# Rengar-Yang/humanoid-gym-with-comments

Measured on AMD Instinct MI355X. Metric: env-steps/sec (whole node) at 4096 envs + PPO iters/sec, 1/2/4/8 MI355X, higher is better.
Workload: dtype f32; 1 GPU; XBot-L flat terrain, 4096 envs/GPU, PPO 24-step rollout (BASELINE configs[1]); envs_per_gpu=4096, num_steps_per_env=24, parallelism=dp1, ppo=2 epochs x 4 minibatches, actor 705-512-256-128-12, critic 219-768-256-128-1, update_graph=one, gemm_table=tuning/tunableop_mi355x_f32.csv

## Files before the change

humanoid-gym-with-comments_amd/csrc/hg_gemm.hip:

```cpp
#include <hip/hip_runtime.h>
#include <stdint.h>

#include <type_traits>

#include "hg_common.h"

namespace {

typedef float f32x16 __attribute__((ext_vector_type(16)));
typedef float f32x4u __attribute__((ext_vector_type(4), aligned(4)));

struct GemmArgs {
  const float* A;
  int64_t lda;
  const float* B;
  int64_t ldb;
  const float* bias;
  const float* Y;
  int64_t ldY;
  float* C;
  int64_t ldc;
  float* colpart;
  int64_t M;
  int N, K;
// ... 676 lines not shown
    epi_input_grad<TM, TN, ELU>(acc, g, m0 + wm0, n0 + wn0, i, h, cs);
#pragma unroll
    for (int n = 0; n < TN; n++) {
      const int cl = wn0 + 32 * n + i;
      cs[n] += __shfl_xor(cs[n], 32);
      if (h == 0) red[(wave % WGM) * BN + cl] = cs[n];
    }
    if (g.colpart) {
      __syncthreads();
      for (int c = tid; c < BN; c += NT) {
        if (n0 + c <= nmax) {
          float sum = 0.f;
#pragma unroll
          for (int w = 0; w < WGM; w++) sum += red[w * BN + c];
          g.colpart[tm_idx * g.N + n0 + c] = sum;
        }
      }
    }
  }
}

template <int BM, int BN, int WGM, int WGN, int KG, bool VEC, int MODE, bool ELU, int IMG = 0, bool APF = false>
__global__ void __launch_bounds__(64 * WGM * WGN) k_gemm_x6(GemmX6Args xa) {
  gemm_x6_body<BM, BN, WGM, WGN, KG, VEC, MODE, ELU, IMG, APF>(xa);
}

template <int BM, int BN, int WGM, int WGN, int KG, bool VEC, int MODE, bool ELU, int IMG = 0, bool APF = false,
          int OCC = 4>
__global__ void __launch_bounds__(64 * WGM * WGN) __attribute__((amdgpu_waves_per_eu(OCC)))
k_gemm_x6_occ(GemmX6Args xa) {
  gemm_x6_body<BM, BN, WGM, WGN, KG, VEC, MODE, ELU, IMG, APF>(xa);
}

constexpr int IMG_MAX = 16;
struct ImageJobs {
  const float* P[IMG_MAX];
  bf16x8* img[IMG_MAX];
  int64_t ld[IMG_MAX], pitch[IMG_MAX];
  int trans[IMG_MAX], R[IMG_MAX], K[IMG_MAX], groups[IMG_MAX];
  int block0[IMG_MAX + 1];
  int njobs;
};

__host__ __device__ inline int64_t img_rows(int64_t R) { return (R + 255) / 256 * 256; }
__host__ __device__ inline int64_t img_chunks(int64_t K) { return (K + 31) / 32 * 2; }

__global__ void __launch_bounds__(256) k_x6_image_jobs(ImageJobs J) {
  const int bid = blockIdx.x;
  int j = 0;
  while (j + 1 < J.njobs && bid >= J.block0[j + 1]) j++;
  const int lb = bid - J.block0[j];
  const int grp = lb % J.groups[j], c = lb / J.groups[j];
  const int r = grp * 128 + (threadIdx.x & 127), h = threadIdx.x >> 7;
  const float* __restrict__ P = J.P[j];
  const int64_t ld = J.ld[j];
  const int R = J.R[j], K = J.K[j];
  const int k0 = c * 16 + 8 * h;
  float v[8];
  if (J.trans[j]) {
#pragma unroll
    for (int q = 0; q < 8; q++) v[q] = (r < R && k0 + q < K) ? P[(int64_t)(k0 + q) * ld + r] : 0.f;
  } else if (r < R && k0 + 8 <= K && ld % 4 == 0 && ((uintptr_t)P & 15) == 0) {
    const float4 a = *reinterpret_cast<const float4*>(P + (int64_t)r * ld + k0);
    const float4 b = *reinterpret_cast<const float4*>(P + (int64_t)r * ld + k0 + 4);
    v[0] = a.x; v[1] = a.y; v[2] = a.z; v[3] = a.w; v[4] = b.x; v[5] = b.y; v[6] = b.z; v[7] = b.w;
  } else {
// ... 21 lines not shown
#define HG_X6I(V, MD, E, I)                                                                                      \
  do {                                                                                                             \
    if constexpr (OCC > 0) hipLaunchKernelGGL((k_gemm_x6_occ<BM, BN, WGM, WGN, KG, V, MD, E, I, APF, OCC>), grid, block, 0, s, xa); \
    else hipLaunchKernelGGL((k_gemm_x6<BM, BN, WGM, WGN, KG, V, MD, E, I, APF>), grid, block, 0, s, xa);             \
  } while (0)
  if (mode == 2) {
    HG_X6I(false, 2, false, 3);
  } else if (mode == 4) {
    if (vec) HG_X6I(true, 4, false, 1);
    else HG_X6I(false, 4, false, 1);
  } else if (img == 3) {
    if (mode == 0) {
      if (elu) HG_X6I(false, 0, true, 3);
      else HG_X6I(false, 0, false, 3);
    } else {
      if (elu) HG_X6I(false, 1, true, 3);
      else HG_X6I(false, 1, false, 3);
    }
  } else if (mode == 0) {
    if (vec && elu) HG_X6I(true, 0, true, 1);
    else if (vec) HG_X6I(true, 0, false, 1);
    else if (elu) HG_X6I(false, 0, true, 1);
    else HG_X6I(false, 0, false, 1);
  } else {
    if (vec && elu) HG_X6I(true, 1, true, 1);
    else if (vec) HG_X6I(true, 1, false, 1);
    else if (elu) HG_X6I(false, 1, true, 1);
    else HG_X6I(false, 1, false, 1);
  }
#undef HG_X6I
  return hipGetLastError() == hipSuccess ? HG_OK : HG_ERR_HIP;
}

int x6_img_dispatch(int tile, int mode, int img, GemmX6Args xa, bool vec, bool elu, hipStream_t s) {
  switch (tile) {
    case 20: return launch_x6_img<128, 128, 2, 2, 1>(mode, img, xa, vec, elu, s);
    case 21: return launch_x6_img<128, 128, 2, 4, 1>(mode, img, xa, vec, elu, s);
    case 22: return launch_x6_img<128, 64, 2, 2, 1>(mode, img, xa, vec, elu, s);
    case 23: return launch_x6_img<64, 64, 2, 2, 1>(mode, img, xa, vec, elu, s);
    case 24: return launch_x6_img<128, 128, 2, 2, 2>(mode, img, xa, vec, elu, s);
    case 25: return launch_x6_img<256, 128, 4, 2, 1>(mode, img, xa, vec, elu, s);
    case 26: return launch_x6_img<128, 128, 2, 4, 2>(mode, img, xa, vec, elu, s);
    case 27: return launch_x6_img<128, 256, 2, 4, 1>(mode, img, xa, vec, elu, s);
    case 28: return launch_x6_img<64, 256, 2, 4, 1>(mode, img, xa, vec, elu, s);
    case 29: return launch_x6_img<64, 64, 2, 2, 1, true>(mode, img, xa, vec, elu, s);
    case 30: return launch_x6_img<256, 128, 4, 2, 1, false, 4>(mode, img, xa, vec, elu, s);
    case 31: return launch_x6_img<128, 64, 2, 2, 1, false, 4>(mode, img, xa, vec, elu, s);
    case 32: return launch_x6_img<128, 128, 2, 4, 1, false, 6>(mode, img, xa, vec, elu, s);
    default: return launch_x6_img<64, 128, 2, 2, 1>(mode, img, xa, vec, elu, s);
  }
}

template <int BM, int BN, int WGM, int WGN, int KG>
int launch_x6(int mode, GemmX6Args xa, bool vec, bool elu, hipStream_t s) {
  GemmArgs& g = xa.g;
  g.tiles_n = (g.N + BN - 1) / BN;
  const int64_t tiles_m = (g.M + BM - 1) / BM;
  g.tiles = tiles_m * g.tiles_n;
  if (mode != 2 && mode != 4) xa.slices = 1;
  if (g.tiles * xa.slices > 0x7fffffff) return HG_ERR_ARG;
  const dim3 grid((unsigned)(g.tiles * xa.slices)), block(64 * WGM * WGN);
#define HG_X6(V, MD, E) hipLaunchKernelGGL((k_gemm_x6<BM, BN, WGM, WGN, KG, V, MD, E>), grid, block, 0, s, xa)
  if (mode == 0) {
    if (vec && elu) HG_X6(true, 0, true);
    else if (vec) HG_X6(true, 0, false);
    else if (elu) HG_X6(false, 0, true);
    else HG_X6(false, 0, false);
  } else if (mode == 1) {
    if (vec && elu) HG_X6(true, 1, true);
    else if (vec) HG_X6(true, 1, false);
    else if (elu) HG_X6(false, 1, true);
    else HG_X6(false, 1, false);
  } else if (mode == 3) {
    if (vec && elu) HG_X6(true, 3, true);
    else if (vec) HG_X6(true, 3, false);
    else if (elu) HG_X6(false, 3, true);
    else HG_X6(false, 3, false);
  } else if (mode == 4) {
    if (vec) HG_X6(true, 4, false);
    else HG_X6(false, 4, false);
  } else {
    HG_X6(false, 2, false);
  }
#undef HG_X6
  return hipGetLastError() == hipSuccess ? HG_OK : HG_ERR_HIP;
}

constexpr int NTILES = 29;
constexpr int NTILES_IMG = 32;
int tile_bm(int tile) {
  if (tile == 25 || tile == 30) return 256;
  return (tile <= 2 || (tile >= 8 && tile <= 10) || tile == 12 || tile == 13 || tile == 16 || tile == 17 ||
          (tile >= 20 && tile <= 22) || tile == 24 || tile == 26 || tile == 27 || tile == 31 || tile == 32)
             ? 128
             : 64;
}

struct WgradArgs {
  const float* A;
  int64_t lda;
  const float* B;
  int64_t ldb;
  float* C;
  int64_t ldc, cstride;
  int M, N;
  int64_t R, kslice;
  int slices, tiles_n;
  int64_t tiles;
};

typedef short s16x4 __attribute__((ext_vector_type(4)));
typedef float f32x2 __attribute__((ext_vector_type(2)));
typedef __bf16 bf16x2 __attribute__((ext_vector_type(2)));

__device__ __forceinline__ uint32_t bf16_pair(f32x2 v) {
  return __builtin_bit_cast(uint32_t, __builtin_convertvector(v, bf16x2));
}
__device__ __forceinline__ f32x2 bf16_pair_f32(uint32_t u) {
  f32x2 r;
  r[0] = __uint_as_float(u << 16);
  r[1] = __uint_as_float(u & 0xffff0000u);
  return r;
}
__device__ __forceinline__ void split3x4(const float v[4], uint2& p0, uint2& p1, uint2& p2) {
// ... 209 lines not shown
    J.pitch[j] = img_rows(prow) * 2;
    J.trans[j] = trans[j];
    J.R[j] = (int)rows[j];
    J.K[j] = (int)K[j];
    J.groups[j] = (int)(img_rows(rows[j]) / 128);
    J.block0[j] = (int)blocks;
    blocks += img_chunks(K[j]) * J.groups[j];
    if (blocks > (int64_t)1 << 30) return HG_ERR_ARG;
  }
  J.block0[njobs] = (int)blocks;
  for (int j = 0; j < njobs;) {
    const int64_t prow = pitch_rows && pitch_rows[j] > 0 ? pitch_rows[j] : rows[j];
    int64_t sum = rows[j];
    int e = j + 1;
    while (e < njobs && pitch_rows && pitch_rows[e] == prow && K[e] == K[j] && sum < prow &&
           (uintptr_t)img[e] == (uintptr_t)img[e - 1] + (uintptr_t)(32 * rows[e - 1])) {
      sum += rows[e];
      e++;
    }
    if (sum != prow) return HG_ERR_ARG;
    for (int b = j; b + 1 < e; b++)
      if (rows[b] % 256) return HG_ERR_ARG;
    j = e;
  }
  hipLaunchKernelGGL(k_x6_image_jobs, dim3((unsigned)blocks), dim3(256), 0, (hipStream_t)stream, J);
  return hipGetLastError() == hipSuccess ? HG_OK : HG_ERR_HIP;
}

extern "C" int hg_gemm_f32_img(int mode, const float* A, int64_t lda, const void* Aimg, const void* Bimg,
                               const float* bias, const float* Y, int64_t ldY, float* C, int64_t ldc, float* colpart,
                               int64_t M, int N, int K, int act, int tile, int64_t aimg_bytes, int64_t bimg_bytes,
                               void* stream) {
  if ((!A && !Aimg) || !Bimg || !C || M <= 0 || N <= 0 || K <= 0 || ldc < N || (mode != 0 && mode != 1) || act < 0 ||
      act > 1 || tile < 19 || tile > NTILES_IMG)
    return HG_ERR_ARG;
  if (!Aimg && lda < K) return HG_ERR_ARG;
  if (bimg_bytes != hg_gemm_x6_image_bytes(N, K) || (Aimg && aimg_bytes != hg_gemm_x6_image_bytes(M, K)))
    return HG_ERR_ARG;
  if (mode == 1 && act == 1 && (!Y || ldY < N)) return HG_ERR_ARG;
  if ((!Aimg && (uintptr_t)A % 4) || (uintptr_t)Aimg % 16 || (uintptr_t)Bimg % 16 || (uintptr_t)C % 4)
    return HG_ERR_ARG;
  const bool vec = !Aimg && lda % 4 == 0 && (uintptr_t)A % 16 == 0;
  const float* a = Aimg ? reinterpret_cast<const float*>(Aimg) : A;
  const int64_t la = Aimg ? img_rows(M) * 2 : lda;
  GemmArgs g{a, la, reinterpret_cast<const float*>(Bimg), img_rows(N) * 2, bias, Y, ldY, C, ldc, colpart, M, N, K, 0, 0};
  GemmX6Args xa{g, 0, 0, 1};
  return x6_img_dispatch(tile, mode, Aimg ? 3 : 1, xa, vec, act == 1, (hipStream_t)stream);
}

extern "C" int hg_gemm_f32_img_split(const float* A, int64_t lda, const void* Bimg, const float* bias,
                                     const float* bias2, float* C, int64_t ldc, float* C2, int64_t ldc2, int nsplit,
                                     int64_t M, int N, int K, int act, int tile, int64_t bimg_bytes, void* stream) {
  if (!A || !Bimg || !C || !C2 || !bias != !bias2 || M <= 0 || N <= 0 || K <= 0 || nsplit <= 0 || nsplit >= N || nsplit % 256 ||
      ldc < nsplit || ldc2 < N - nsplit || lda < K || act < 0 || act > 1 || tile < 19 || tile > NTILES_IMG)
    return HG_ERR_ARG;
  if (bimg_bytes != hg_gemm_x6_image_bytes(N, K)) return HG_ERR_ARG;
  if ((uintptr_t)A % 4 || (uintptr_t)Bimg % 16 || (uintptr_t)C % 4 || (uintptr_t)C2 % 4) return HG_ERR_ARG;
  const bool vec = lda % 4 == 0 && (uintptr_t)A % 16 == 0;
  GemmArgs g{A, lda, reinterpret_cast<const float*>(Bimg), img_rows(N) * 2, bias, nullptr, 0, C, ldc, nullptr, M, N, K,
             0, 0, C2, ldc2, nsplit, bias2};
  GemmX6Args xa{g, 0, 0, 1};
  return x6_img_dispatch(tile, 0, 1, xa, vec, act == 1, (hipStream_t)stream);
}

extern "C" int hg_gemm_wgrad_img(const void* Aimg, const void* Bimg, float* C, int64_t ldc, int64_t cstride, int64_t M,
                                 int N, int64_t K, int slices, int tile, int64_t aimg_bytes, int64_t bimg_bytes,
                                 void* stream) {
  if (!Aimg || !Bimg || !C || M <= 0 || N <= 0 || K <= 0 || K > 0x7fffffff || ldc < N || slices < 1 || tile < 19 ||
      tile > NTILES)
    return HG_ERR_ARG;
  if (aimg_bytes != hg_gemm_x6_image_bytes(M, K) || bimg_bytes != hg_gemm_x6_image_bytes(N, K)) return HG_ERR_ARG;
  if (slices > 1 && cstride < M * (int64_t)ldc) return HG_ERR_ARG;
  if ((uintptr_t)Aimg % 16 || (uintptr_t)Bimg % 16 || (uintptr_t)C % 4) return HG_ERR_ARG;
  GemmArgs g{reinterpret_cast<const float*>(Aimg), img_rows(M) * 2, reinterpret_cast<const float*>(Bimg),
             img_rows(N) * 2, nullptr, nullptr, 0, C, ldc, nullptr, M, N, (int)K, 0, 0};
  const int64_t kslice = ((K + slices - 1) / slices + 31) & ~(int64_t)31;
  GemmX6Args xa{g, kslice, cstride, slices};
  return x6_img_dispatch(tile, 2, 3, xa, false, false, (hipStream_t)stream);
}

extern "C" int hg_gemm_tile(int mode, int64_t M, int N, int K) {
  (void)mode;
  (void)K;
  const int64_t t16 = ((M + 127) / 128) * ((N + 63) / 64);
  return t16 >= 768 ? 16 : 5;
}

extern "C" int64_t hg_gemm_colpart_rows(int64_t M, int tile) {
  if (tile < 1 || tile > NTILES_IMG) return -1;
  const int bm = tile_bm(tile);
  return (M + bm - 1) / bm;
}

extern "C" int hg_gemm_f32(int mode, const float* A, int64_t lda, const float* B, int64_t ldb, const float* bias,
                           const float* Y, int64_t ldY, float* C, int64_t ldc, float* colpart, int64_t M, int N, int K,
                           int act, int tile, void* stream) {
  if (tile == 30) tile = 25;
  else if (tile == 31) tile = 22;
  else if (tile == 32) tile = 21;
  if (!A || !B || !C || M <= 0 || N <= 0 || K <= 0 || lda < K || ldc < N || mode < 0 || mode > 3 || mode == 2 ||
      act < 0 || act > 1 || tile < 1 || tile > NTILES)
    return HG_ERR_ARG;
  if (mode == 3 && tile < 19) return HG_ERR_ARG;
  if ((mode == 0 || mode == 3) && ldb < K) return HG_ERR_ARG;
  if (mode == 1 && ldb < N) return HG_ERR_ARG;
  if ((mode == 1 || mode == 3) && act == 1 && (!Y || ldY < N)) return HG_ERR_ARG;
  if ((uintptr_t)A % 4 || (uintptr_t)B % 4 || (uintptr_t)C % 4) return HG_ERR_ARG;
  const bool vec = lda % 4 == 0 && (uintptr_t)A % 16 == 0 &&
                   (mode == 1 || (ldb % 4 == 0 && (uintptr_t)B % 16 == 0));
  GemmArgs g{A, lda, B, ldb, bias, Y, ldY, C, ldc, colpart, M, N, K, 0, 0};
  hipStream_t s = (hipStream_t)stream;
  const bool elu = act == 1;
  switch (tile) {
    case 1: return launch<128, 128, 2, 2, 32, 0>(mode, g, vec, elu, s);
    case 2: return launch<128, 64, 2, 2, 32, 0>(mode, g, vec, elu, s);
    case 3: return launch<64, 128, 2, 2, 32, 0>(mode, g, vec, elu, s);
    case 4: return launch<64, 64, 2, 2, 32, 0>(mode, g, vec, elu, s);
    case 5: return launch<64, 64, 2, 2, 32, 1>(mode, g, vec, elu, s);
    case 6: return launch<64, 64, 2, 2, 64, 0>(mode, g, vec, elu, s);
    case 7: return launch<64, 64, 2, 2, 64, 1>(mode, g, vec, elu, s);
    case 8: return launch<128, 64, 4, 2, 32, 1>(mode, g, vec, elu, s);
    case 9: return launch<128, 128, 2, 4, 32, 1>(mode, g, vec, elu, s);
    case 10: return launch<128, 64, 2, 2, 64, 1>(mode, g, vec, elu, s);
    case 11: return launch<64, 64, 2, 2, 16, 1>(mode, g, vec, elu, s);
    case 12: return launch<128, 128, 2, 4, 16, 1>(mode, g, vec, elu, s);
    case 13: return launch<128, 64, 4, 2, 16, 1>(mode, g, vec, elu, s);
    case 14: return launch<64, 128, 2, 2, 16, 1>(mode, g, vec, elu, s);
    case 15: return launch<64, 64, 2, 2, 32, 1, 1>(mode, g, vec, elu, s);
    case 16: return launch<128, 64, 4, 2, 32, 1, 1>(mode, g, vec, elu, s);
    case 17: return launch<128, 128, 2, 4, 32, 1, 1>(mode, g, vec, elu, s);
    case 18: return launch<64, 64, 2, 2, 16, 1, 1>(mode, g, vec, elu, s);
    default: break;
// ... 146 lines not shown
  const int64_t kslice = hg_gemm_splitk_kslice(K, slices);
  if ((slices - 1) * kslice >= K) return HG_ERR_ARG;
  if (ws_floats < slices * M * (int64_t)N) return HG_ERR_ARG;
  if ((uintptr_t)A % 4 || (uintptr_t)B % 4 || (uintptr_t)C % 4 || (uintptr_t)bias % 4 || (uintptr_t)ws % 16)
    return HG_ERR_ARG;
  const int64_t threads = M * ((N + 3) / 4);
  if ((threads + 255) / 256 > 0x7fffffff) return HG_ERR_ARG;
  hipStream_t s = (hipStream_t)stream;
  GemmArgs g{A, lda, B, ldb, nullptr, nullptr, 0, ws, N, nullptr, M, N, K, 0, 0};
  GemmX6Args xa{g, kslice, M * (int64_t)N, slices};
  const bool vec = lda % 4 == 0 && ldb % 4 == 0 && (uintptr_t)A % 16 == 0 && (uintptr_t)B % 16 == 0;
  const bool elu = act == 1;
  const int md = 4;
  int rc;
  switch (tile) {
    case 20: rc = launch_x6<128, 128, 2, 2, 1>(md, xa, vec, elu, s); break;
    case 21: rc = launch_x6<128, 128, 2, 4, 1>(md, xa, vec, elu, s); break;
    case 22: rc = launch_x6<128, 64, 2, 2, 1>(md, xa, vec, elu, s); break;
    case 23: rc = launch_x6<64, 64, 2, 2, 1>(md, xa, vec, elu, s); break;
    case 24: rc = launch_x6<128, 128, 2, 2, 2>(md, xa, vec, elu, s); break;
    case 25: rc = launch_x6<256, 128, 4, 2, 1>(md, xa, vec, elu, s); break;
    case 26: rc = launch_x6<128, 128, 2, 4, 2>(md, xa, vec, elu, s); break;
    case 27: rc = launch_x6<128, 256, 2, 4, 1>(md, xa, vec, elu, s); break;
    default: rc = launch_x6<64, 256, 2, 4, 1>(md, xa, vec, elu, s); break;
  }
  if (rc != HG_OK) return rc;
  return splitk_finish(ws, bias, C, ldc, M, N, slices, elu, s);
}

extern "C" int hg_gemm_f32_splitk_img(const float* A, int64_t lda, const void* Bimg, int64_t bimg_bytes,
                                      const float* bias, float* C, int64_t ldc, float* ws, int64_t ws_floats,
                                      int64_t M, int N, int K, int act, int tile, int slices, void* stream) {
  if (!A || !Bimg || !bias || !C || !ws || M <= 0 || N <= 0 || K <= 0 || lda < K || ldc < N || act < 0 || act > 1 ||
      tile < 19 || tile > NTILES_IMG || tile == 24 || tile == 26 || tile == 29 || slices < 2 || slices > 16)
    return HG_ERR_ARG;
  if (bimg_bytes != hg_gemm_x6_image_bytes(N, K)) return HG_ERR_ARG;
  const int64_t kslice = hg_gemm_splitk_kslice(K, slices);
  if ((slices - 1) * kslice >= K) return HG_ERR_ARG;
  if (ws_floats < slices * M * (int64_t)N) return HG_ERR_ARG;
  if ((uintptr_t)A % 4 || (uintptr_t)Bimg % 16 || (uintptr_t)C % 4 || (uintptr_t)bias % 4 || (uintptr_t)ws % 16)
    return HG_ERR_ARG;
  if ((M * ((N + 3) / 4) + 255) / 256 > 0x7fffffff) return HG_ERR_ARG;
  hipStream_t s = (hipStream_t)stream;
  GemmArgs g{A, lda, reinterpret_cast<const float*>(Bimg), img_rows(N) * 2, nullptr, nullptr, 0, ws, N, nullptr, M, N,
             K, 0, 0};
  GemmX6Args xa{g, kslice, M * (int64_t)N, slices};
  const bool vec = lda % 4 == 0 && (uintptr_t)A % 16 == 0;
  const int rc = x6_img_dispatch(tile, 4, 1, xa, vec, false, s);
  if (rc != HG_OK) return rc;
  return splitk_finish(ws, bias, C, ldc, M, N, slices, act == 1, s);
}
```

humanoid-gym-with-comments_amd/humanoid/_native.py:

```python
import ctypes
import json
import os

import numpy as np

PKG_ROOT = os.path.dirname(os.path.dirname(os.path.abspath(__file__)))
LIB_PATH = os.environ.get("HG_LIB") or os.path.join(PKG_ROOT, "csrc", "libhgsim.so")
MODEL_PATH = os.path.join(PKG_ROOT, "model", "xbotl_model.json")

HG_MAX_BODIES = 16
HG_MAX_DOF = 12
HG_MAX_CONTACTS = 24
HG_MAX_CAPSULES = 12
HG_MAX_PAIRS = 16
HG_NUM_REWARDS = 22
HG_LAMW = HG_MAX_CONTACTS * 3 + HG_MAX_PAIRS * 3 + 2 * HG_MAX_DOF

f32 = ctypes.c_float
i32 = ctypes.c_int32


class HgModel(ctypes.Structure):
    _fields_ = [
        ("num_bodies", i32), ("num_dof", i32), ("num_contacts", i32), ("num_foot_contacts", i32),
# ... 84 lines not shown
        raise ValueError(f"depth: need 0 <= near_clip < far_clip < inf, got {cam.near_clip}, {cam.far_clip}")
    if not (0.0 < cam.horizontal_fov_deg < 180.0):
        raise ValueError(f"depth.horizontal_fov must be inside (0, 180), got {cam.horizontal_fov_deg}")
    if not (cam.noise >= 0.0):
        raise ValueError(f"depth noise must be >= 0, got {cam.noise}")
    return cam


TENSOR_IDS = [
    "ROOT_STATE", "DOF_POS", "DOF_VEL", "CONTACT_FORCES", "RIGID_STATE", "TORQUES", "ACTIONS",
    "LAST_ACTIONS", "LAST_LAST_ACTIONS", "LAST_DOF_VEL", "LAST_ROOT_VEL", "COMMANDS", "OBS_BUF",
    "PRIV_BUF", "REW_BUF", "RESET_BUF", "TIME_OUT_BUF", "EPISODE_LENGTH", "EPISODE_SUMS",
    "FEET_AIR_TIME", "LAST_CONTACTS", "FEET_HEIGHT", "LAST_FEET_Z", "ENV_FRICTION", "BODY_MASS",
    "PUSH_FORCE", "PUSH_TORQUE", "BASE_LIN_VEL", "BASE_ANG_VEL", "PROJ_GRAVITY", "BASE_EULER",
    "REF_DOF_POS", "ENV_ORIGINS", "EP_STATS", "CONTACT_LAMBDA", "NONFINITE", "TERRAIN_LEVEL", "TERRAIN_TYPE",
    "EP_STATS_RING", "ROWS_DROPPED", "ENV_ROWS", "ENV_ORDER",
    "KP_SCALE", "KD_SCALE", "ARMATURE_ADD", "CMD_RANGE_X", "CURRICULUM_RING",
]
EP_RING = 64
T = {name: i for i, name in enumerate(TENSOR_IDS)}

EXPORTS = ["hg_arena_bytes", "hg_create", "hg_destroy", "hg_last_error", "hg_tensor", "hg_step",
           "hg_post", "hg_set_rollout_sink", "hg_ep_stats_slot", "hg_obs_head", "hg_obs_window_advance", "hg_update_cfg", "hg_reset_masked",
           "hg_set_command_range_x", "hg_publish_terrain_level", "hg_set_dof_state_indexed", "hg_set_root_state_indexed",
           "hg_set_root_state", "hg_set_env_props", "hg_set_actuator_props",
           "hg_measure_heights", "hg_render_depth", "hg_gae_scan", "hg_gae_stats_len", "hg_gae_normalize", "hg_adam_step", "hg_adam_chunk", "hg_kl_mean", "hg_kl_lr_rule",
           "hg_rollout_act", "hg_rollout_act_head", "hg_rollout_act_tail", "hg_rollout_env", "hg_gather_rows", "hg_gather_rows_ex", "hg_gather_stacked", "hg_ppo_loss", "hg_ppo_loss_lr", "hg_ppo_loss_scratch", "hg_ppo_loss_backward",
           "hg_mirror_rows", "hg_sym_loss", "hg_sym_loss_scratch", "hg_sym_loss_backward",
           "hg_mlp_act_backward", "hg_mlp_act_backward_scratch", "hg_colsum_jobs", "hg_linear_skinny_supported",
           "hg_linear_skinny_forward", "hg_linear_skinny_backward", "hg_linear_skinny_backward_scratch",
           "hg_mlp_act_backward_bf16", "hg_linear_skinny_forward_bf16", "hg_linear_skinny_backward_bf16",
           "hg_cast_bf16_jobs", "hg_linear_act_forward", "hg_linear_act_tile", "hg_gemm_f32", "hg_gemm_tile",
           "hg_gemm_colpart_rows", "hg_gemm_f32_wgrad", "hg_gemm_x6_image_bytes", "hg_gemm_x6_image_jobs", "hg_gemm_x6_image_jobs_pitched", "hg_gemm_wgrad_img",
           "hg_gemm_f32_img", "hg_gemm_f32_img_split", "hg_gemm_splitk_kslice", "hg_gemm_f32_splitk", "hg_gemm_f32_splitk_img", "hg_linear_skinny_backward_act", "hg_linear_skinny_colpart_rows", "hg_version",
           "hg_source_hash"]

_LIB = None

DTYPE_CODES = {"float32": 0, "float16": 1, "bfloat16": 2}


class GatherTable(ctypes.Structure):
    _fields_ = [("src", ctypes.c_void_p), ("dst", ctypes.c_void_p), ("width", ctypes.c_int64),
                ("src_dtype", ctypes.c_int32), ("dst_dtype", ctypes.c_int32)]


def source_hash(pkg_root=PKG_ROOT):
    import hashlib
    try:
        with open(os.path.join(pkg_root, "Makefile")) as f:
            srcs = next(ln.split("=", 1)[1].split() for ln in f if ln.startswith("SRCS ="))
        h = hashlib.sha256()
        for rel in srcs + ["csrc/hg_common.h", "../include/hgsim.h"]:
            with open(os.path.join(pkg_root, rel), "rb") as f:
                h.update(f.read())
        return h.hexdigest()[:16]
    except (OSError, StopIteration):
        return None


def load_library(path=LIB_PATH):
    if not os.path.exists(path):
        raise RuntimeError(
            f"hg_sim HIP library not found at {path}: build it with `python -c 'import __graft_entry__ as g; g.build()'` "
            "(there is no CPU fallback on the product path)")
    import torch
    L = ctypes.CDLL(path, mode=ctypes.RTLD_GLOBAL)
# ... 140 lines not shown
    L.hg_gemm_f32_wgrad.restype = ctypes.c_int
    L.hg_gemm_f32_wgrad.argtypes = [vp, ctypes.c_int64, vp, ctypes.c_int64, vp, ctypes.c_int64, ctypes.c_int64,
                                    ctypes.c_int64, ctypes.c_int, ctypes.c_int64, ctypes.c_int, ctypes.c_int, ctypes.c_int,
                                    vp]
    L.hg_gemm_x6_image_bytes.restype = ctypes.c_int64
    L.hg_gemm_x6_image_bytes.argtypes = [ctypes.c_int64, ctypes.c_int64]
    L.hg_gemm_x6_image_jobs.restype = ctypes.c_int
    L.hg_gemm_x6_image_jobs.argtypes = [ctypes.POINTER(vp), ctypes.POINTER(ctypes.c_int64), ctypes.POINTER(ctypes.c_int),
                                        ctypes.POINTER(ctypes.c_int64), ctypes.POINTER(ctypes.c_int64),
                                        ctypes.POINTER(vp), ctypes.c_int, vp]
    L.hg_gemm_x6_image_jobs_pitched.restype = ctypes.c_int
    L.hg_gemm_x6_image_jobs_pitched.argtypes = [ctypes.POINTER(vp), ctypes.POINTER(ctypes.c_int64),
                                                ctypes.POINTER(ctypes.c_int), ctypes.POINTER(ctypes.c_int64),
                                                ctypes.POINTER(ctypes.c_int64), ctypes.POINTER(vp),
                                                ctypes.POINTER(ctypes.c_int64), ctypes.c_int, vp]
    L.hg_gemm_f32_img_split.restype = ctypes.c_int
    L.hg_gemm_f32_img_split.argtypes = [vp, ctypes.c_int64, vp, vp, vp, vp, ctypes.c_int64, vp, ctypes.c_int64, ctypes.c_int,
                                        ctypes.c_int64, ctypes.c_int, ctypes.c_int, ctypes.c_int, ctypes.c_int,
                                        ctypes.c_int64, vp]
    L.hg_gemm_splitk_kslice.restype = ctypes.c_int64
    L.hg_gemm_splitk_kslice.argtypes = [ctypes.c_int, ctypes.c_int]
    L.hg_gemm_f32_splitk.restype = ctypes.c_int
    L.hg_gemm_f32_splitk.argtypes = [vp, ctypes.c_int64, vp, ctypes.c_int64, vp, vp, ctypes.c_int64, vp, ctypes.c_int64,
                                     ctypes.c_int64, ctypes.c_int, ctypes.c_int, ctypes.c_int, ctypes.c_int, ctypes.c_int,
                                     vp]
    L.hg_gemm_f32_splitk_img.restype = ctypes.c_int
    L.hg_gemm_f32_splitk_img.argtypes = [vp, ctypes.c_int64, vp, ctypes.c_int64, vp, vp, ctypes.c_int64, vp,
                                         ctypes.c_int64, ctypes.c_int64, ctypes.c_int, ctypes.c_int, ctypes.c_int,
                                         ctypes.c_int, ctypes.c_int, vp]
    L.hg_gemm_f32_img.restype = ctypes.c_int
    L.hg_gemm_f32_img.argtypes = [ctypes.c_int, vp, ctypes.c_int64, vp, vp, vp, vp, ctypes.c_int64, vp, ctypes.c_int64,
                                  vp, ctypes.c_int64, ctypes.c_int, ctypes.c_int, ctypes.c_int, ctypes.c_int,
                                  ctypes.c_int64, ctypes.c_int64, vp]
    L.hg_gemm_wgrad_img.restype = ctypes.c_int
    L.hg_gemm_wgrad_img.argtypes = [vp, vp, vp, ctypes.c_int64, ctypes.c_int64, ctypes.c_int64, ctypes.c_int,
                                    ctypes.c_int64, ctypes.c_int, ctypes.c_int, ctypes.c_int64, ctypes.c_int64, vp]
    L.hg_gemm_tile.restype = ctypes.c_int
    L.hg_gemm_tile.argtypes = [ctypes.c_int, ctypes.c_int64, ctypes.c_int, ctypes.c_int]
    L.hg_gemm_colpart_rows.restype = ctypes.c_int64
    L.hg_gemm_colpart_rows.argtypes = [ctypes.c_int64, ctypes.c_int]
    L.hg_linear_skinny_backward_act.restype = ctypes.c_int
    L.hg_linear_skinny_backward_act.argtypes = [vp, vp, ctypes.c_int64, vp, vp, vp, ctypes.c_int64, ctypes.c_int,
                                                ctypes.c_int, vp, vp]
    L.hg_linear_skinny_colpart_rows.restype = ctypes.c_int64
    L.hg_linear_skinny_colpart_rows.argtypes = [ctypes.c_int64]
    L.hg_version.restype = ctypes.c_char_p
    L.hg_version.argtypes = []
    return L


def lib():
    global _LIB
    if _LIB is None:
        _LIB = load_library()
    return _LIB


def check(status, handle=None):
    if status != 0:
        msg = lib().hg_last_error(handle)
        raise RuntimeError(f"hg_sim error {status}: {msg.decode() if msg else '?'}")


def stream_ptr(device):
    import torch
    return ctypes.c_void_p(torch.cuda.current_stream(device).cuda_stream)
# ... 79 lines not shown
```

humanoid-gym-with-comments_amd/humanoid/algo/ppo/hg_mlp.py:

```python
import contextlib
import ctypes
import os

import torch
import torch.nn as nn
import torch.nn.functional as F

from humanoid import _native as N


def fusable(net):
    mods = list(net)
    if not mods or not isinstance(mods[-1], nn.Linear):
        return False
    for i, m in enumerate(mods):
        want = nn.Linear if i % 2 == 0 else nn.ELU
        if not isinstance(m, want):
            return False
        if isinstance(m, nn.ELU) and (m.alpha != 1.0 or m.inplace):
            return False
        if isinstance(m, nn.Linear) and m.bias is None:
            return False
    return True

# ... 455 lines not shown


class _MLP(torch.autograd.Function):
    @staticmethod
    def forward(ctx, x, *params):
        n = len(params) // 2
        fimg, ctx.dximg = _forward_images(params, n, x.shape[0], x.device, any(ctx.needs_input_grad))
        acts = []
        h = _mlp_forward_layers(x, params, n, fimg, 0, acts)
        ctx.save_for_backward(*acts, *params[0::2])
        ctx.n = n
        return h

    @staticmethod
    def backward(ctx, g):
        n = ctx.n
        saved = ctx.saved_tensors
        ins, Ws = saved[:n], saved[n:]
        red = _Reductions() if DEFER_REDUCTIONS else None
        grads, gx = _mlp_backward_layers(g, ins, Ws, n, ctx.dximg, ctx.needs_input_grad[0], red)
        if red is not None:
            red.launch(ins[0].device)
        ctx.dximg = None
        return (gx, *grads)


_PAIR_FWD = {(705, 640): [(8192, 0), (_BIG, 30)]}
if os.environ.get("HG_OCC_TILES", "1") == "0":
    _PAIR_FWD[(705, 640)] = [(8192, 0), (_BIG, 25)]
    _GEMM_DX[(256, 768)] = [(_BIG, 22)]
    _GEMM_DX[(256, 512)] = [(_BIG, 28)]
    _GEMM_DX[(128, 256)] = [(_BIG, 16)]
    _GEMM_FWD[(219, 768)] = [(32768, 21), (_BIG, 20)]
PAIR_FIRST = os.environ.get("HG_PAIR_FIRST", "1") != "0"


def pair_ok(net_a, net_b, rows):
    if not (PAIR_FIRST and GEMM and X6_IMAGE and fusable(net_a) and fusable(net_b)):
        return False
    la, lb = net_a[0], net_b[0]
    if len(net_a) < 3 or len(net_b) < 3 or la.in_features != lb.in_features or la.out_features % 256:
        return False
    ps = (la.weight, lb.weight, la.bias, lb.bias)
    if not all(p.is_cuda and p.dtype == torch.float32 and p.is_contiguous() for p in ps):
        return False
    return _route(_PAIR_FWD, rows, la.in_features, la.out_features + lb.out_features) >= X6_TILE0


class _MLPPair(torch.autograd.Function):
    @staticmethod
    def forward(ctx, x, na, *params):
        pa, pb = params[:2 * na], params[2 * na:]
        nb = len(pb) // 2
        rows, K = x.shape
        Wa, Wb = pa[0], pb[0]
        ma, mb = Wa.shape[0], Wb.shape[0]
        key = ("stack", Wa.data_ptr(), Wb.data_ptr())
        img = _SCOPE.get(key) if _SCOPE is not None else None
        if img is None:
            img = x6_images([("stack", (Wa, Wb), K)], x.device)[0]
        tile = _route(_PAIR_FWD, rows, K, ma + mb)
        ha = torch.empty(rows, ma, dtype=torch.float32, device=x.device)
        hb = torch.empty(rows, mb, dtype=torch.float32, device=x.device)
        rc = N.lib().hg_gemm_f32_img_split(x.data_ptr(), x.stride(0), img.data_ptr(), pa[1].data_ptr(), pb[1].data_ptr(),
                                           ha.data_ptr(), ma,
                                           hb.data_ptr(), mb, ma, rows, ma + mb, K, 1, tile,
# ... 277 lines not shown
```

include/hgsim.h:

```cpp
#ifndef HGSIM_H
#define HGSIM_H

#include <stddef.h>
#include <stdint.h>

#ifdef __cplusplus
extern "C" {
#endif

#define HG_OK 0
#define HG_ERR_ARG 1
#define HG_ERR_HIP 2
#define HG_ERR_STATE 3

#define HG_MAX_BODIES 16
#define HG_MAX_DOF 12
#define HG_MAX_CONTACTS 24
#define HG_MAX_CAPSULES 12
#define HG_MAX_PAIRS 16
#define HG_NUM_REWARDS 22
#define HG_MAX_TENSORS 32
#define HG_MAX_HEIGHT_POINTS 1024
#define HG_LAMW (HG_MAX_CONTACTS * 3 + HG_MAX_PAIRS * 3 + 2 * HG_MAX_DOF)

// ... 286 lines not shown
int64_t hg_linear_skinny_colpart_rows(int64_t rows);
int hg_mlp_act_backward_bf16(const uint16_t* gy, const uint16_t* y, uint16_t* gh, int64_t rows, int width,
                             float* grad_bias, float* scratch ,
                             void* stream);
int hg_linear_skinny_forward_bf16(const uint16_t* x, int64_t ldx, const float* W, const float* b, float* y,
                                  int64_t rows, int n, int k, void* stream);
int hg_linear_skinny_backward_bf16(const float* gh, const uint16_t* h, int64_t ldh, const float* W, uint16_t* dx,
                                   float* grad_wb, int64_t rows, int n, int k,
                                   float* scratch , void* stream);
int hg_cast_bf16_jobs(const float* const* src, uint16_t* const* dst, const int64_t* count, int njobs, void* stream);
int hg_colsum_jobs(const float* const* src, float* const* dst, const int64_t* width, const int* parts, int njobs,
                   void* stream);

int hg_linear_act_forward(const float* x, int64_t ldx, const float* W, const float* b, float* y, int64_t ldy,
                          int64_t rows, int n, int k, int act, int tile, void* stream);
int hg_linear_act_tile(int64_t rows, int n, int k);

int hg_gemm_f32(int mode, const float* A, int64_t lda, const float* B, int64_t ldb, const float* bias, const float* Y,
                int64_t ldY, float* C, int64_t ldc, float* colpart, int64_t M, int N, int K, int act, int tile,
                void* stream);
int hg_gemm_tile(int mode, int64_t M, int N, int K);
int hg_gemm_f32_wgrad(const float* A, int64_t lda, const float* B, int64_t ldb, float* C, int64_t ldc,
                      int64_t cstride, int64_t M, int N, int64_t K, int slices, int kmajor, int tile, void* stream);
int64_t hg_gemm_colpart_rows(int64_t M, int tile);
int64_t hg_gemm_x6_image_bytes(int64_t rows, int64_t K);
int hg_gemm_x6_image_jobs(const float* const* P, const int64_t* ld, const int* trans, const int64_t* rows,
                          const int64_t* K, void* const* img, int njobs, void* stream);
int hg_gemm_x6_image_jobs_pitched(const float* const* P, const int64_t* ld, const int* trans, const int64_t* rows,
                                  const int64_t* K, void* const* img, const int64_t* pitch_rows, int njobs,
                                  void* stream);
int hg_gemm_f32_img(int mode, const float* A, int64_t lda, const void* Aimg, const void* Bimg, const float* bias,
                    const float* Y, int64_t ldY, float* C, int64_t ldc, float* colpart, int64_t M, int N, int K,
                    int act, int tile, int64_t aimg_bytes, int64_t bimg_bytes, void* stream);
int hg_gemm_f32_img_split(const float* A, int64_t lda, const void* Bimg, const float* bias, const float* bias2,
                          float* C, int64_t ldc, float* C2, int64_t ldc2, int nsplit, int64_t M, int N, int K, int act,
                          int tile, int64_t bimg_bytes, void* stream);
int hg_gemm_wgrad_img(const void* Aimg, const void* Bimg, float* C, int64_t ldc, int64_t cstride, int64_t M, int N,
                      int64_t K, int slices, int tile, int64_t aimg_bytes, int64_t bimg_bytes, void* stream);
int64_t hg_gemm_splitk_kslice(int K, int slices);
int hg_gemm_f32_splitk(const float* A, int64_t lda, const float* B, int64_t ldb, const float* bias, float* C,
                       int64_t ldc, float* ws, int64_t ws_floats, int64_t M, int N, int K, int act, int tile,
                       int slices, void* stream);
int hg_gemm_f32_splitk_img(const float* A, int64_t lda, const void* Bimg, int64_t bimg_bytes, const float* bias,
                           float* C, int64_t ldc, float* ws, int64_t ws_floats, int64_t M, int N, int K, int act,
                           int tile, int slices, void* stream);

const char* hg_version(void);
const char* hg_source_hash(void);

#ifdef __cplusplus
}
#endif
#endif
```

Before: 5.747 million env-steps/s.

## Add multi-stage pipelined x6 bf16-split GEMM kernel with async LDS ring

Adds a new GEMM kernel variant (tiles 34-36) for the fp32-emulated bf16x3 MFMA path. It streams B through a 3-deep LDS ring using global_load_lds DMA and prefetches A into registers several K-chunks ahead, with explicit vmcnt waits. Some forward and input-grad routes in the MLP tables now use it, enabled by default behind an environment flag. The goal is to hide global-memory latency behind MFMA work. In exchange it uses more LDS and hand-tuned waitcnt logic that could be fragile.

New measurement: 5.739 million env-steps/s, median of 2. Within noise of the previous version (-0.1%).

```diff
diff --git a/humanoid-gym-with-comments_amd/csrc/hg_gemm.hip b/humanoid-gym-with-comments_amd/csrc/hg_gemm.hip
--- a/humanoid-gym-with-comments_amd/csrc/hg_gemm.hip
+++ b/humanoid-gym-with-comments_amd/csrc/hg_gemm.hip
@@ -732,6 +732,254 @@
   gemm_x6_body<BM, BN, WGM, WGN, KG, VEC, MODE, ELU, IMG, APF>(xa);
 }
 
+typedef float f32x4 __attribute__((ext_vector_type(4)));
+
+template <int N>
+__device__ __forceinline__ void wait_vm() {
+  static_assert(N >= 0 && N < 64, "vmcnt is a 6-bit field");
+  asm volatile("s_waitcnt vmcnt(%0)" ::"n"(N) : "memory");
+}
+
+template <int PER, int NB, int D>
+__device__ __forceinline__ void pipe_wait(int f, int t) {
+  const int key = 2 * f + t;
+  if (key == 1) wait_vm<NB>();
+  else if (key == 2) wait_vm<PER>();
+  else if (D > 2 && key == 3) wait_vm<PER + NB>();
+  else if (D > 2 && key == 4) wait_vm<2 * PER>();
+  else wait_vm<0>();
+}
+
+template <int BM, int BN, int WGM, int WGN, int MODE, bool ELU, int NS, int D>
+__device__ __forceinline__ void gemm_x6_pipe_body(const GemmX6Args& xa) {
+  constexpr int NW = WGM * WGN, NT = 64 * NW;
+  constexpr int TM = BM / WGM / 32, TN = BN / WGN / 32;
+  constexpr int PA = BM * 2, PB = BN * 2;
+  constexpr int SA = 3 * PA, SB = 3 * PB;
+  constexpr int NSA = 2;
+  constexpr int LDS_SLOTS = NSA * SA + NS * SB;
+  constexpr int ITEMS = BM * 2;
+  constexpr int UB = 3 * (BN / 32);
+  constexpr int NB = (UB + NW - 1) / NW;
+  constexpr int NA = 2;
+  static_assert(MODE == 0 || MODE == 1, "forward and input grad");
+  static_assert(TM >= 1 && TN >= 1 && BM == 32 * TM * WGM && BN == 32 * TN * WGN, "wave tiling");
+  static_assert(ITEMS <= NT && ITEMS % 64 == 0, "at most one A item per thread, whole waves");
+  static_assert(D == 3 && NS >= 3, "ring depth");
+  static_assert(LDS_SLOTS * 16 <= 160 * 1024, "LDS");
+  static_assert(LDS_SLOTS * 4 >= WGM * BN, "epilogue reduction buffer fits the rings");
+  __shared__ __attribute__((aligned(16))) bf16x8 lds[LDS_SLOTS];
+  bf16x8* const ldsB = lds + NSA * SA;
+  const GemmArgs& g = xa.g;
+
+  const int tid = threadIdx.x;
+  const int lane = tid & 63, wave = tid >> 6;
+  const int i = lane & 31, h = lane >> 5;
+  const unsigned nb = gridDim.x;
+  unsigned L = blockIdx.x;
+  if ((nb & 7u) == 0) L = (blockIdx.x & 7u) * (nb >> 3) + (blockIdx.x >> 3);
+  if ((int64_t)L >= g.tiles) return;
+  const int64_t tile = (int64_t)L;
+  const int64_t tm_idx = tile / g.tiles_n;
+  const int64_t m0 = tm_idx * BM;
+  const int n0 = (int)(tile % g.tiles_n) * BN;
+  const int wm0 = (wave % WGM) * (32 * TM), wn0 = (wave / WGM) * (32 * TN);
+  const int64_t mmax = g.M - 1;
+  const int nmax = g.N - 1;
+
+  f32x16 acc[TM][TN];
+#pragma unroll
+  for (int m = 0; m < TM; m++)
+#pragma unroll
+    for (int n = 0; n < TN; n++) acc[m][n] = (f32x16)0.f;
+
+  const int nfull = g.K >> 4;
+  const bool has_tail = (g.K & 15) != 0;
+  const int nch = nfull + (has_tail ? 1 : 0);
+
+  const bf16x8* bsrc = reinterpret_cast<const bf16x8*>(g.B) + (int64_t)n0 * 2 + lane;
+  auto dma_b = [&](int c, bf16x8* S) {
+    constexpr int U = BN / 32;
+#pragma unroll
+    for (int t = 0; t < NB; t++) {
+      int q = wave + t * NW;
+      if (UB % NW != 0) q = min(q, UB - 1);
+      const int u = q % U, p = q / U;
+      const bf16x8* src = bsrc + ((int64_t)c * 3 + p) * g.ldb + u * 64;
+      __builtin_amdgcn_global_load_lds(src, (__attribute__((address_space(3))) void*)(S + p * PB + u * 64), 16, 0, 0);
+    }
+  };
+  struct ASet {
+    f32x4 x, y;
+  };
+  ASet sA[D], sT;
+  const int ar = tid >> 1, ap = tid & 1;
+  const int kt = nfull * 16 + 8 * ap;
+  const bool a_on = ITEMS == NT || tid < ITEMS;
+  const float* aptr = g.A + min<int64_t>(m0 + ar, mmax) * g.lda + 8 * ap;
+  auto load_a = [&](ASet& S, int c) {
+    if (a_on) {
+      const float* p = aptr + (int64_t)c * 16;
+      asm volatile("global_load_dwordx4 %0, %2, off\n\tglobal_load_dwordx4 %1, %2, off offset:16"
+                   : "=&v"(S.x), "=&v"(S.y)
+                   : "v"(p)
+                   : "memory");
+    }
+  };
+  auto store_a = [&](const ASet& S, bf16x8* St) {
+    if (a_on) {
+      const float v[8] = {S.x[0], S.x[1], S.x[2], S.x[3], S.y[0], S.y[1], S.y[2], S.y[3]};
+      bf16x8 x0, x1, x2;
+      split3x8(v, x0, x1, x2);
+      const int sl = x6_slot(BM, 0, ar, ap);
+      St[sl] = x0;
+      St[PA + sl] = x1;
+      St[2 * PA + sl] = x2;
+    }
+  };
+  struct Frag {
+    bf16x8 a[3][TM], b[3][TN];
+  };
+  auto frag = [&](int j, Frag& F) {
+    const bf16x8* ca = lds + (j % NSA) * SA;
+    const bf16x8* cb = ldsB + (j % NS) * SB;
+#pragma unroll
+    for (int p = 0; p < 3; p++) {
+#pragma unroll
+      for (int m = 0; m < TM; m++) F.a[p][m] = ca[p * PA + x6_slot(BM, 0, wm0 + 32 * m + i, h)];
+#pragma unroll
+      for (int n = 0; n < TN; n++) F.b[p][n] = cb[p * PB + x6_slot(BN, 0, wn0 + 32 * n + i, h)];
+    }
+  };
+  auto mma = [&](const Frag& F) {
+#pragma unroll
+    for (int m = 0; m < TM; m++)
+#pragma unroll
+      for (int n = 0; n < TN; n++) {
+        acc[m][n] = __builtin_amdgcn_mfma_f32_32x32x16_bf16(F.a[2][m], F.b[0][n], acc[m][n], 0, 0, 0);
+        acc[m][n] = __builtin_amdgcn_mfma_f32_32x32x16_bf16(F.a[1][m], F.b[1][n], acc[m][n], 0, 0, 0);
+        acc[m][n] = __builtin_amdgcn_mfma_f32_32x32x16_bf16(F.a[0][m], F.b[2][n], acc[m][n], 0, 0, 0);
+        acc[m][n] = __builtin_amdgcn_mfma_f32_32x32x16_bf16(F.a[1][m], F.b[0][n], acc[m][n], 0, 0, 0);
+        acc[m][n] = __builtin_amdgcn_mfma_f32_32x32x16_bf16(F.a[0][m], F.b[1][n], acc[m][n], 0, 0, 0);
+        acc[m][n] = __builtin_amdgcn_mfma_f32_32x32x16_bf16(F.a[0][m], F.b[0][n], acc[m][n], 0, 0, 0);
+      }
+  };
+  auto consume = [&](int n1, int hi, ASet& S, auto steady) {
+    {
+      bf16x8* St = lds + (n1 % NSA) * SA;
+      if (decltype(steady)::value) {
+        if (ITEMS == NT || a_on) wait_vm<NB + NA>();
+        else wait_vm<NB>();
+        asm volatile("" : "+v"(S.x), "+v"(S.y)::"memory");
+        store_a(S, St);
+      } else if (has_tail && n1 == nch - 1) {
+        asm volatile("" : "+v"(sT.x), "+v"(sT.y)::"memory");
+        ASet Z;
+#pragma unroll
+        for (int q = 0; q < 4; q++) {
+          Z.x[q] = kt + q < g.K ? sT.x[q] : 0.f;
+          Z.y[q] = kt + 4 + q < g.K ? sT.y[q] : 0.f;
+        }
+        store_a(Z, St);
+        wait_vm<0>();
+      } else {
+        const int t = (has_tail && hi == nch - 1 && hi > n1) ? 1 : 0;
+        const int f = max(hi - n1, 0) - t;
+        if (ITEMS == NT || a_on) pipe_wait<NB + NA, NB, 2>(f, t);
+        else pipe_wait<NB, NB, 2>(f, t);
+        asm volatile("" : "+v"(S.x), "+v"(S.y)::"memory");
+        store_a(S, St);
+      }
+    }
+  };
+  auto sync = [&]() {
+    asm volatile("s_waitcnt lgkmcnt(0)" ::: "memory");
+    __builtin_amdgcn_s_barrier();
+  };
+  auto issue = [&](int j, ASet& S, auto steady) {
+    dma_b(j, ldsB + (j % NS) * SB);
+    if (decltype(steady)::value || j < nfull) load_a(S, j);
+  };
+  auto step = [&](int c, const Frag& Fcur, Frag& Fnext, ASet& Sissue, ASet& Scons, auto steady) {
+    if (decltype(steady)::value || c + 3 < nch) issue(c + 3, Sissue, steady);
+    if (decltype(steady)::value || c + 1 < nch) frag(c + 1, Fnext);
+    mma(Fcur);
+    if (decltype(steady)::value || c + 2 < nch) consume(c + 2, min(c + 3, nch - 1), Scons, steady);
+    sync();
+  };
+  const std::true_type STEADY;
+  const std::false_type EDGE;
+
+  if (has_tail) {
+    const float* p = aptr - 8 * ap;
+#pragma unroll
+    for (int q = 0; q < 4; q++) {
+      sT.x[q] = p[min(kt + q, g.K - 1)];
+      sT.y[q] = p[min(kt + 4 + q, g.K - 1)];
+    }
+  }
+  issue(0, sA[0], EDGE);
+  if (1 < nch) issue(1, sA[1], EDGE);
+  consume(0, min(1, nch - 1), sA[0], EDGE);
+  if (2 < nch) issue(2, sA[0], EDGE);
+  if (1 < nch) consume(1, min(2, nch - 1), sA[1], EDGE);
+  sync();
+  Frag F0, F1;
+  frag(0, F0);
+  sync();
+  int c = 0;
+  for (; c + 4 < nfull; c += 2) {
+    step(c, F0, F1, sA[1], sA[0], STEADY);
+    step(c + 1, F1, F0, sA[0], sA[1], STEADY);
+  }
+  for (; c < nch; c += 2) {
+    step(c, F0, F1, sA[1], sA[0], EDGE);
+    if (c + 1 < nch) step(c + 1, F1, F0, sA[0], sA[1], EDGE);
+  }
+
+  if (MODE == 0) {
+    float* Cs = g.C;
+    int64_t ldcs = g.ldc;
+    int cshift = 0;
+    const float* bs = g.bias;
+    if (g.nsplit > 0 && n0 >= g.nsplit) {
+      Cs = g.C2;
+      ldcs = g.ldc2;
+      cshift = g.nsplit;
+      bs = g.bias2;
+    }
+    if (g.bias) epi_forward<TM, TN, ELU, true>(acc, g, Cs, m0 + wm0, n0 + wn0, i, h, ldcs, cshift, bs);
+    else epi_forward<TM, TN, ELU, false>(acc, g, Cs, m0 + wm0, n0 + wn0, i, h, ldcs, cshift, bs);
+  } else {
+    float* red = reinterpret_cast<float*>(lds);
+    float cs[TN];
+    epi_input_grad<TM, TN, ELU>(acc, g, m0 + wm0, n0 + wn0, i, h, cs);
+#pragma unroll
+    for (int n = 0; n < TN; n++) {
+      const int cl = wn0 + 32 * n + i;
+      cs[n] += __shfl_xor(cs[n], 32);
+      if (h == 0) red[(wave % WGM) * BN + cl] = cs[n];
+    }
+    if (g.colpart) {
+      __syncthreads();
+      for (int c2 = tid; c2 < BN; c2 += NT) {
+        if (n0 + c2 <= nmax) {
+          float sum = 0.f;
+#pragma unroll
+          for (int w = 0; w < WGM; w++) sum += red[w * BN + c2];
+          g.colpart[tm_idx * g.N + n0 + c2] = sum;
+        }
+      }
+    }
+  }
+}
+
+template <int BM, int BN, int WGM, int WGN, int MODE, bool ELU, int NS, int D, int OCC>
+__global__ void __launch_bounds__(64 * WGM * WGN) __attribute__((amdgpu_waves_per_eu(OCC)))
+k_gemm_x6_pipe(GemmX6Args xa) {
+  gemm_x6_pipe_body<BM, BN, WGM, WGN, MODE, ELU, NS, D>(xa);
+}
+
 constexpr int IMG_MAX = 16;
 struct ImageJobs {
   const float* P[IMG_MAX];
@@ -819,7 +1067,47 @@
   return hipGetLastError() == hipSuccess ? HG_OK : HG_ERR_HIP;
 }
 
+template <int BM, int BN, int WGM, int WGN, int NS, int D, int OCC>
+int launch_x6_pipe(int mode, GemmX6Args xa, bool elu, hipStream_t s) {
+  GemmArgs& g = xa.g;
+  g.tiles_n = (g.N + BN - 1) / BN;
+  const int64_t tiles_m = (g.M + BM - 1) / BM;
+  g.tiles = tiles_m * g.tiles_n;
+  xa.slices = 1;
+  if (g.tiles > 0x7fffffff) return HG_ERR_ARG;
+  const dim3 grid((unsigned)g.tiles), block(64 * WGM * WGN);
+#define HG_X6P(MD, E) hipLaunchKernelGGL((k_gemm_x6_pipe<BM, BN, WGM, WGN, MD, E, NS, D, OCC>), grid, block, 0, s, xa)
+  if (mode == 0) {
+    if (elu) HG_X6P(0, true);
+    else HG_X6P(0, false);
+  } else {
+    if (elu) HG_X6P(1, true);
+    else HG_X6P(1, false);
+  }
+#undef HG_X6P
+  return hipGetLastError() == hipSuccess ? HG_OK : HG_ERR_HIP;
+}
+
+#ifndef HG_PIPE_D
+#define HG_PIPE_D 3
+#endif
+constexpr int PIPE_D = HG_PIPE_D;
+constexpr int PIPE_NS_25 = 3, PIPE_NS_22 = 3, PIPE_NS_21 = 3;
+
+int x6_base_tile(int tile) {
+  if (tile == 30 || tile == 34) return 25;
+  if (tile == 31 || tile == 35) return 22;
+  if (tile == 32 || tile == 36) return 21;
+  return tile;
+}
+
 int x6_img_dispatch(int tile, int mode, int img, GemmX6Args xa, bool vec, bool elu, hipStream_t s) {
+  if (tile >= 34 && tile <= 36) {
+    if (img != 1 || (mode != 0 && mode != 1)) tile = x6_base_tile(tile);
+    else if (tile == 34) return launch_x6_pipe<256, 128, 4, 2, PIPE_NS_25, PIPE_D, 2>(mode, xa, elu, s);
+    else if (tile == 35) return launch_x6_pipe<128, 64, 2, 2, PIPE_NS_22, PIPE_D, 3>(mode, xa, elu, s);
+    else return launch_x6_pipe<128, 128, 2, 4, PIPE_NS_21, PIPE_D, 2>(mode, xa, elu, s);
+  }
   switch (tile) {
     case 20: return launch_x6_img<128, 128, 2, 2, 1>(mode, img, xa, vec, elu, s);
     case 21: return launch_x6_img<128, 128, 2, 4, 1>(mode, img, xa, vec, elu, s);
@@ -874,9 +1162,11 @@
 }
 
 constexpr int NTILES = 29;
-constexpr int NTILES_IMG = 32;
+constexpr int NTILES_IMG = 36;
+inline bool img_tile_ok(int tile) { return tile >= 19 && tile <= NTILES_IMG && tile != 33; }
 int tile_bm(int tile) {
-  if (tile == 25 || tile == 30) return 256;
+  tile = x6_base_tile(tile);
+  if (tile == 25) return 256;
   return (tile <= 2 || (tile >= 8 && tile <= 10) || tile == 12 || tile == 13 || tile == 16 || tile == 17 ||
           (tile >= 20 && tile <= 22) || tile == 24 || tile == 26 || tile == 27 || tile == 31 || tile == 32)
              ? 128
@@ -1152,7 +1442,7 @@
                                int64_t M, int N, int K, int act, int tile, int64_t aimg_bytes, int64_t bimg_bytes,
                                void* stream) {
   if ((!A && !Aimg) || !Bimg || !C || M <= 0 || N <= 0 || K <= 0 || ldc < N || (mode != 0 && mode != 1) || act < 0 ||
-      act > 1 || tile < 19 || tile > NTILES_IMG)
+      act > 1 || !img_tile_ok(tile))
     return HG_ERR_ARG;
   if (!Aimg && lda < K) return HG_ERR_ARG;
   if (bimg_bytes != hg_gemm_x6_image_bytes(N, K) || (Aimg && aimg_bytes != hg_gemm_x6_image_bytes(M, K)))
@@ -1172,7 +1462,7 @@
                                      const float* bias2, float* C, int64_t ldc, float* C2, int64_t ldc2, int nsplit,
                                      int64_t M, int N, int K, int act, int tile, int64_t bimg_bytes, void* stream) {
   if (!A || !Bimg || !C || !C2 || !bias != !bias2 || M <= 0 || N <= 0 || K <= 0 || nsplit <= 0 || nsplit >= N || nsplit % 256 ||
-      ldc < nsplit || ldc2 < N - nsplit || lda < K || act < 0 || act > 1 || tile < 19 || tile > NTILES_IMG)
+      ldc < nsplit || ldc2 < N - nsplit || lda < K || act < 0 || act > 1 || !img_tile_ok(tile))
     return HG_ERR_ARG;
   if (bimg_bytes != hg_gemm_x6_image_bytes(N, K)) return HG_ERR_ARG;
   if ((uintptr_t)A % 4 || (uintptr_t)Bimg % 16 || (uintptr_t)C % 4 || (uintptr_t)C2 % 4) return HG_ERR_ARG;
@@ -1207,17 +1497,22 @@
 }
 
 extern "C" int64_t hg_gemm_colpart_rows(int64_t M, int tile) {
-  if (tile < 1 || tile > NTILES_IMG) return -1;
+  if (tile < 1 || tile > NTILES_IMG || tile == 33) return -1;
   const int bm = tile_bm(tile);
   return (M + bm - 1) / bm;
+}
+
+extern "C" int hg_gemm_x6_pipe_shape(int tile, int* stages, int* depth) {
+  if (tile < 34 || tile > 36 || !stages || !depth) return HG_ERR_ARG;
+  *stages = tile == 34 ? PIPE_NS_25 : tile == 35 ? PIPE_NS_22 : PIPE_NS_21;
+  *depth = PIPE_D;
+  return HG_OK;
 }
 
 extern "C" int hg_gemm_f32(int mode, const float* A, int64_t lda, const float* B, int64_t ldb, const float* bias,
                            const float* Y, int64_t ldY, float* C, int64_t ldc, float* colpart, int64_t M, int N, int K,
                            int act, int tile, void* stream) {
-  if (tile == 30) tile = 25;
-  else if (tile == 31) tile = 22;
-  else if (tile == 32) tile = 21;
+  tile = x6_base_tile(tile);
   if (!A || !B || !C || M <= 0 || N <= 0 || K <= 0 || lda < K || ldc < N || mode < 0 || mode > 3 || mode == 2 ||
       act < 0 || act > 1 || tile < 1 || tile > NTILES)
     return HG_ERR_ARG;
@@ -1430,7 +1725,7 @@
                                       const float* bias, float* C, int64_t ldc, float* ws, int64_t ws_floats,
                                       int64_t M, int N, int K, int act, int tile, int slices, void* stream) {
   if (!A || !Bimg || !bias || !C || !ws || M <= 0 || N <= 0 || K <= 0 || lda < K || ldc < N || act < 0 || act > 1 ||
-      tile < 19 || tile > NTILES_IMG || tile == 24 || tile == 26 || tile == 29 || slices < 2 || slices > 16)
+      !img_tile_ok(tile) || tile == 24 || tile == 26 || tile == 29 || slices < 2 || slices > 16)
     return HG_ERR_ARG;
   if (bimg_bytes != hg_gemm_x6_image_bytes(N, K)) return HG_ERR_ARG;
   const int64_t kslice = hg_gemm_splitk_kslice(K, slices);
diff --git a/humanoid-gym-with-comments_amd/humanoid/_native.py b/humanoid-gym-with-comments_amd/humanoid/_native.py
--- a/humanoid-gym-with-comments_amd/humanoid/_native.py
+++ b/humanoid-gym-with-comments_amd/humanoid/_native.py
@@ -140,7 +140,7 @@
            "hg_mlp_act_backward_bf16", "hg_linear_skinny_forward_bf16", "hg_linear_skinny_backward_bf16",
            "hg_cast_bf16_jobs", "hg_linear_act_forward", "hg_linear_act_tile", "hg_gemm_f32", "hg_gemm_tile",
            "hg_gemm_colpart_rows", "hg_gemm_f32_wgrad", "hg_gemm_x6_image_bytes", "hg_gemm_x6_image_jobs", "hg_gemm_x6_image_jobs_pitched", "hg_gemm_wgrad_img",
-           "hg_gemm_f32_img", "hg_gemm_f32_img_split", "hg_gemm_splitk_kslice", "hg_gemm_f32_splitk", "hg_gemm_f32_splitk_img", "hg_linear_skinny_backward_act", "hg_linear_skinny_colpart_rows", "hg_version",
+           "hg_gemm_f32_img", "hg_gemm_x6_pipe_shape", "hg_gemm_f32_img_split", "hg_gemm_splitk_kslice", "hg_gemm_f32_splitk", "hg_gemm_f32_splitk_img", "hg_linear_skinny_backward_act", "hg_linear_skinny_colpart_rows", "hg_version",
            "hg_source_hash"]
 
 _LIB = None
@@ -347,6 +347,8 @@
     L.hg_gemm_f32_img.argtypes = [ctypes.c_int, vp, ctypes.c_int64, vp, vp, vp, vp, ctypes.c_int64, vp, ctypes.c_int64,
                                   vp, ctypes.c_int64, ctypes.c_int, ctypes.c_int, ctypes.c_int, ctypes.c_int,
                                   ctypes.c_int64, ctypes.c_int64, vp]
+    L.hg_gemm_x6_pipe_shape.restype = ctypes.c_int
+    L.hg_gemm_x6_pipe_shape.argtypes = [ctypes.c_int, ctypes.POINTER(ctypes.c_int), ctypes.POINTER(ctypes.c_int)]
     L.hg_gemm_wgrad_img.restype = ctypes.c_int
     L.hg_gemm_wgrad_img.argtypes = [vp, vp, vp, ctypes.c_int64, ctypes.c_int64, ctypes.c_int64, ctypes.c_int,
                                     ctypes.c_int64, ctypes.c_int, ctypes.c_int, ctypes.c_int64, ctypes.c_int64, vp]
diff --git a/humanoid-gym-with-comments_amd/humanoid/algo/ppo/hg_mlp.py b/humanoid-gym-with-comments_amd/humanoid/algo/ppo/hg_mlp.py
--- a/humanoid-gym-with-comments_amd/humanoid/algo/ppo/hg_mlp.py
+++ b/humanoid-gym-with-comments_amd/humanoid/algo/ppo/hg_mlp.py
@@ -511,6 +511,13 @@
     _GEMM_DX[(256, 512)] = [(_BIG, 28)]
     _GEMM_DX[(128, 256)] = [(_BIG, 16)]
     _GEMM_FWD[(219, 768)] = [(32768, 21), (_BIG, 20)]
+_X6_PIPE_ROUTES = [(_GEMM_FWD, (512, 256), _BIG, 35), (_GEMM_FWD, (768, 256), 32768, 35),
+                   (_GEMM_DX, (256, 512), _BIG, 35), (_GEMM_DX, (256, 768), _BIG, 35)]
+X6_PIPE = os.environ.get("HG_X6_PIPE", "1") != "0"
+if X6_PIPE and os.environ.get("HG_OCC_TILES", "1") != "0":
+    for _table, _key, _rows, _tile in _X6_PIPE_ROUTES:
+        _table[_key] = [(r, _tile if r == _rows else t) for r, t in _table[_key]]
+    _GEMM_FWD[(780, 768)] = _GEMM_FWD[(219, 768)]
 PAIR_FIRST = os.environ.get("HG_PAIR_FIRST", "1") != "0"
 
 
diff --git a/include/hgsim.h b/include/hgsim.h
--- a/include/hgsim.h
+++ b/include/hgsim.h
@@ -342,6 +342,7 @@
 int hg_gemm_f32_img(int mode, const float* A, int64_t lda, const void* Aimg, const void* Bimg, const float* bias,
                     const float* Y, int64_t ldY, float* C, int64_t ldc, float* colpart, int64_t M, int N, int K,
                     int act, int tile, int64_t aimg_bytes, int64_t bimg_bytes, void* stream);
+int hg_gemm_x6_pipe_shape(int tile, int* stages, int* depth);
 int hg_gemm_f32_img_split(const float* A, int64_t lda, const void* Bimg, const float* bias, const float* bias2,
                           float* C, int64_t ldc, float* C2, int64_t ldc2, int nsplit, int64_t M, int N, int K, int act,
                           int tile, int64_t bimg_bytes, void* stream);
```
